# jtstrader/mercer-research

Measured on AMD Instinct MI355X. Metric: training images/sec, MNIST-shape 28x28x1 batch=256, at 1/2/4/8 MI355X, higher is better.
Workload: dtype f32

## Files before the change

mercer_research_amd/csrc/dense_xcd.hpp:

```cpp
#pragma once

#include "dense_p2.hpp"
#include "dense_p2_dp.hpp"
#include "dp_push.hpp"

namespace rcn {

constexpr int kXcdWorkers = 32, kXcdThreads = 512, kXcdFlagStride = 32;
constexpr int kXcdSl = 2;

template <typename T>
struct XcdBufsT {
    T* slab;
    T* d1;
    T* a1;
    T* d2;
    T* loss;
    T* a2;
    T* d3;
    T* fragimg;
    unsigned* flagA;
    unsigned* flagB;
    unsigned* flagT;
    unsigned* xcc;
    unsigned* flagD;
    unsigned* errd;
    unsigned* done;
    unsigned* cw;
    unsigned* cdone;
    long long* phase;
};
using XcdBufs = XcdBufsT<float>;

inline int xcd_na(const NetDesc& nd) { return (pipe_slices(nd) + kXcdSl - 1) / kXcdSl; }
inline bool xcd_two_hidden(const NetDesc& nd) {
    return nd.L == 3 && nd.dims[1] <= kP2H && nd.dims[2] <= kP2C && nd.dims[3] <= kP2C && pipe_slices(nd) <= kP2MaxSlices;
}
inline bool xcd_one_hidden(const NetDesc& nd) {
    return nd.L == 2 && nd.dims[1] <= kP2H && nd.dims[2] <= kP2C && pipe_slices(nd) <= kP2MaxSlices;
}
constexpr int kXcdMaxB = 256;
constexpr int kXcdMaxB64 = 256;
inline int xcd_max_b(size_t esz) { return esz == 8 ? kXcdMaxB64 : kXcdMaxB; }
inline int xcd_bt(size_t B) { return B <= 32 ? 32 : B <= 64 ? 64 : B <= 128 ? 128 : 256; }
inline bool xcd_supported(const NetDesc& nd, size_t B, size_t esz = 4) {
    return (xcd_one_hidden(nd) || xcd_two_hidden(nd)) && B >= 1 && B <= (size_t)xcd_max_b(esz) && xcd_na(nd) + pipe_extra_wgs(nd) <= kXcdWorkers &&
           pipe_extra_wgs(nd) <= 8;
}
inline int xcd_workers(const NetDesc& nd, int BT) {
    const int roles = xcd_na(nd) + pipe_extra_wgs(nd), groups = BT / kP2Ts;
    return roles > groups ? roles : groups;
}
inline size_t xcd_buf_bytes(const NetDesc& nd, size_t BT, size_t esz = 4) {
    const size_t NS = BT / kP2Ts, NA = (size_t)xcd_na(nd);
    return (NS * NA * kP2Ts * kP2H + 2 * BT * kP2H + 3 * BT * kP2C + NS + (size_t)kP3BFrag * 64) * esz +
           (size_t)(4 * kXcdWorkers + 8) * kXcdFlagStride * sizeof(unsigned) + 512 + 1024;
}
constexpr int kXcdD1Ld = 48;
template <typename T, int BT> constexpr bool xcd_red_aliased() { return sizeof(T) == 8 && BT >= 128; }
template <typename T, int BT> constexpr bool xcd_single_buffer() { return sizeof(T) == 8 && BT >= 256; }
constexpr size_t xcd_lds_floats(int BT, bool red_aliased = false, bool single = false) {
    return (single ? 1 : 2) * (size_t)kXcdSl * BT * 16 + (size_t)(single ? BT / 2 : BT) * kXcdD1Ld + (red_aliased ? 0 : (size_t)kDenseWaves * kMtp * kRedTile) +
           (size_t)kXcdSl * 16 * kP2H + (size_t)kP2BWaves * 64 * 4 + kP2H * kLd + 3 * kP2C * kLd + 4 * 64 + 64;
}
template <typename T, int BT> constexpr size_t xcd_lds_bytes() { return xcd_lds_floats(BT, xcd_red_aliased<T, BT>(), xcd_single_buffer<T, BT>()) * sizeof(T); }
static_assert(xcd_lds_bytes<double, 128>() + 64 <= 160 * 1024 && xcd_lds_bytes<float, 256>() + 64 <= 160 * 1024 && xcd_lds_bytes<double, 256>() + 64 <= 160 * 1024,
              "k_xcd_epoch: LDS of the largest instantiations");
static_assert((size_t)2 * kXcdSl * 128 * 16 >= (size_t)kDenseWaves * kMtp * kRedTile, "k_xcd_epoch: the partials fit the batch buffers they are laid over");

#ifdef RCN_STAMPS
#define XSTAMP(i) do { if (j == nb - 2 && lane == 0) g_rcn_stamps[0][w][i] = __builtin_amdgcn_s_memrealtime(); } while (0)
#define XCLOCK(k) do { if (lane == 0 && wave == 0) { g_rcn_stamps[1][w][2 * (k)] = __builtin_amdgcn_s_memtime(); g_rcn_stamps[1][w][2 * (k) + 1] = __builtin_amdgcn_s_memrealtime(); } } while (0)
#else
#define XSTAMP(i) do { } while (0)
#define XCLOCK(k) do { } while (0)
#endif
#if defined(RCN_STAMPS) && defined(RCN_STAMPS_TAIL)
#define XSTAMP_TAIL(i) XSTAMP(i)
#define XSTAMP_FWD(i) do { } while (0)
#else
#define XSTAMP_TAIL(i) do { } while (0)
#define XSTAMP_FWD(i) XSTAMP(i)
#endif

using xu4 = __attribute__((ext_vector_type(4))) unsigned;
#define XCD_RSRC(ptr, bytes) __builtin_amdgcn_make_buffer_rsrc((void*)(ptr), 0, (int)(bytes), 0x00020000)
template <typename T> __device__ inline typename Vec4<T>::type xcd_ld4(__amdgpu_buffer_rsrc_t r, int byte_off);
template <> __device__ inline Vec4<float>::type xcd_ld4<float>(__amdgpu_buffer_rsrc_t r, int byte_off) {
    const xu4 v = __builtin_amdgcn_raw_buffer_load_b128(r, byte_off, 0, 16);
    Vec4<float>::type f;
    __builtin_memcpy(&f, &v, 16);
    return f;
}
template <> __device__ inline Vec4<double>::type xcd_ld4<double>(__amdgpu_buffer_rsrc_t r, int byte_off) {
    const xu4 v[2] = {__builtin_amdgcn_raw_buffer_load_b128(r, byte_off, 0, 16), __builtin_amdgcn_raw_buffer_load_b128(r, byte_off + 16, 0, 16)};
    Vec4<double>::type f;
    __builtin_memcpy(&f, v, 32);
    return f;
}
__device__ inline float xcd_ld1_at(__amdgpu_buffer_rsrc_t r, int lane_off, int uniform_off) {
    const unsigned v = __builtin_amdgcn_raw_buffer_load_b32(r, lane_off, uniform_off, 16);
    float f;
    __builtin_memcpy(&f, &v, 4);
    return f;
}
template <typename T> __device__ inline T xcd_ld1(__amdgpu_buffer_rsrc_t r, int byte_off);
template <> __device__ inline float xcd_ld1<float>(__amdgpu_buffer_rsrc_t r, int byte_off) {
    const unsigned v = __builtin_amdgcn_raw_buffer_load_b32(r, byte_off, 0, 16);
    float f;
    __builtin_memcpy(&f, &v, 4);
    return f;
}
template <> __device__ inline double xcd_ld1<double>(__amdgpu_buffer_rsrc_t r, int byte_off) {
    typedef unsigned xu2 __attribute__((ext_vector_type(2)));
    const xu2 v = __builtin_amdgcn_raw_buffer_load_b64(r, byte_off, 0, 16);
    double f;
    __builtin_memcpy(&f, &v, 8);
    return f;
}
__device__ inline void xcd_drain() { asm volatile("s_waitcnt vmcnt(0)" ::: "memory"); }
__device__ inline void xcd_flag(unsigned* f, unsigned tag) { __hip_atomic_store(f, tag, __ATOMIC_RELAXED, __HIP_MEMORY_SCOPE_WORKGROUP); }
__device__ inline void xcd_flag_wt(unsigned* f, unsigned v) { __hip_atomic_store(f, v, __ATOMIC_RELAXED, __HIP_MEMORY_SCOPE_AGENT); }

enum XcdSite : unsigned {
    kXcdSitePlacement = 1,
    kXcdSiteTailFlag = 2,
    kXcdSiteSlabFlag = 3,
    kXcdSiteDeltaFlag = 4,
    kXcdSitePushOwner = 5,
    kXcdSitePushMember = 6,
    kXcdSitePushTail = 7,
    kXcdSitePushCost = 8,
    kXcdSiteClosing = 9,
};
constexpr int kXcdRecWords = 12;
#ifdef RCN_AB_RAISE_INLINE
__device__ inline void xcd_raise(unsigned* err_host, unsigned* err_dev, unsigned code, unsigned site, int worker, int step, unsigned launch,
                                 unsigned long long missing, unsigned tag, int rank = 0, int world = 1, int xsel = 0, int nw = 0) {
#else
__device__ __attribute__((noinline)) void xcd_raise(unsigned* err_host, unsigned* err_dev, unsigned code, unsigned site, int worker, int step, unsigned launch,
                                                    unsigned long long missing, unsigned tag, int rank = 0, int world = 1, int xsel = 0, int nw = 0) {
#endif
    unsigned expect = 0u;
    if (!__hip_atomic_compare_exchange_strong(err_dev, &expect, code, __ATOMIC_RELAXED, __ATOMIC_RELAXED, __HIP_MEMORY_SCOPE_AGENT)) return;
    unsigned id;
    asm volatile("s_getreg_b32 %0, hwreg(HW_REG_XCC_ID)" : "=s"(id));
    const unsigned rec[kXcdRecWords] = {site, (unsigned)worker, (unsigned)step, launch & 0x3fffffffu, (unsigned)missing, (unsigned)(missing >> 32), tag, id & 0xfu,
                                        (unsigned)rank, (unsigned)world, (unsigned)xsel, (unsigned)nw};
#pragma unroll
    for (int i = 0; i < kXcdRecWords; ++i) __hip_atomic_store(err_host + 4 + i, rec[i], __ATOMIC_RELAXED, __HIP_MEMORY_SCOPE_SYSTEM);
    __hip_atomic_store(err_host, code, __ATOMIC_RELEASE, __HIP_MEMORY_SCOPE_SYSTEM);
}

__device__ inline void xcd_barrier_lds() { asm volatile("s_waitcnt lgkmcnt(0)\n\ts_barrier" ::: "memory"); }

__device__ inline unsigned long long xcd_wait(const unsigned* f0, int n0, const unsigned* f1, int n1, unsigned tag, long long timeout, const unsigned* err) {
    const int lane = threadIdx.x & 63;
    const unsigned* p = lane < n0 ? f0 + lane * kXcdFlagStride : (lane < n0 + n1 ? f1 + (lane - n0) * kXcdFlagStride : nullptr);
    long long t0 = 0;
    for (unsigned it = 0;; ++it) {
        const unsigned f = p ? __hip_atomic_load(p, __ATOMIC_RELAXED, __HIP_MEMORY_SCOPE_AGENT) : tag;
        if (__all((int)(f - tag) >= 0)) return 0ull;
        if ((it & 255u) == 255u) {
            const long long now = wall_clock64();
            if (t0 == 0) t0 = now;
            else if (now - t0 > timeout || __hip_atomic_load(err, __ATOMIC_RELAXED, __HIP_MEMORY_SCOPE_AGENT) != 0u) return __ballot((int)(f - tag) < 0);
        }
    }
}
__device__ inline unsigned long long xcd_wait_some(const unsigned* f0, int first, int stride, int n, unsigned tag, long long timeout, const unsigned* err) {
    const int prod = first + (int)(threadIdx.x & 63) * stride;
    const unsigned* p = prod < n ? f0 + prod * kXcdFlagStride : nullptr;
    long long t0 = 0;
    for (unsigned it = 0;; ++it) {
        const unsigned f = p ? __hip_atomic_load(p, __ATOMIC_RELAXED, __HIP_MEMORY_SCOPE_AGENT) : tag;
        if (__all((int)(f - tag) >= 0)) return 0ull;
        if ((it & 255u) == 255u) {
            const long long now = wall_clock64();
            if (t0 == 0) t0 = now;
            else if (now - t0 > timeout || __hip_atomic_load(err, __ATOMIC_RELAXED, __HIP_MEMORY_SCOPE_AGENT) != 0u) return __ballot((int)(f - tag) < 0);
        }
    }
}
__device__ inline unsigned long long xcd_missing(unsigned long long lanes, int first, int stride) {
    unsigned long long missing = 0ull;
    for (; lanes; lanes &= lanes - 1ull) missing |= 1ull << (first + __builtin_ctzll(lanes) * stride);
    return missing;
}
struct XcdTopMiss { unsigned site; unsigned long long producers; };
__host__ __device__ constexpr XcdTopMiss xcd_top_missing(unsigned long long lanes, int na, int nt) {
    const unsigned long long slab = lanes & ((1ull << na) - 1ull), tail = (lanes >> na) & ((1ull << nt) - 1ull);
    return slab != 0ull ? XcdTopMiss{kXcdSiteSlabFlag, slab} : XcdTopMiss{kXcdSiteTailFlag, tail};
}
static_assert(xcd_top_missing(0x2ull, 25, 3).site == kXcdSiteSlabFlag && xcd_top_missing(0x2ull, 25, 3).producers == 0x2ull, "only a slab part missing");
static_assert(xcd_top_missing(5ull << 25, 25, 3).site == kXcdSiteTailFlag && xcd_top_missing(5ull << 25, 25, 3).producers == 0x5ull, "only tail tiles missing, NT = 3");
static_assert(xcd_top_missing((4ull << 25) | 0x1000002ull, 25, 3).site == kXcdSiteSlabFlag && xcd_top_missing((4ull << 25) | 0x1000002ull, 25, 3).producers == 0x1000002ull,
              "both missing: the slab site, the slab producers only");
static_assert(xcd_top_missing(0x21ull << 25, 25, 6).site == kXcdSiteTailFlag && xcd_top_missing(0x21ull << 25, 25, 6).producers == 0x21ull, "tail tiles 0 and 5 of NT = 6");
static_assert(xcd_top_missing(0x3full << 2, 2, 6).site == kXcdSiteTailFlag && xcd_top_missing(0x3full << 2, 2, 6).producers == 0x3full, "every tail tile of NT = 6 behind NA = 2");
static_assert(xcd_top_missing((1ull << 31) | 1ull, 29, 3).site == kXcdSiteSlabFlag && xcd_top_missing((1ull << 31) | 1ull, 29, 3).producers == 1ull, "NA = 29: the last tail lane is lane 31");
static_assert(xcd_top_missing(1ull << 28, 29, 3).site == kXcdSiteSlabFlag && xcd_top_missing(1ull << 29, 29, 3).site == kXcdSiteTailFlag &&
              xcd_top_missing(1ull << 29, 29, 3).producers == 1ull, "the boundary between the two tables");

constexpr unsigned kXcdPoison = 0x10000u;
__device__ inline bool xcd_commit(unsigned* cw, int NW, long long timeout, const unsigned* err, bool& gave_up, unsigned& seen) {
    unsigned v = __hip_atomic_fetch_add(cw, 1u, __ATOMIC_RELAXED, __HIP_MEMORY_SCOPE_AGENT) + 1u;
    long long t0 = 0;
    gave_up = false;
    for (unsigned it = 0;; ++it) {
        if (v & kXcdPoison) { seen = v; return false; }
        if ((int)(v & 0xffffu) == NW) { seen = v; return true; }
        if ((it & 63u) == 63u) {
            const long long now = wall_clock64();
            if (t0 == 0) t0 = now;
            else if (now - t0 > timeout || __hip_atomic_load(err, __ATOMIC_RELAXED, __HIP_MEMORY_SCOPE_AGENT) != 0u) {
                for (;;) {
                    if (v & kXcdPoison) { seen = v; return false; }
                    if ((int)(v & 0xffffu) == NW) { seen = v; return true; }
                    unsigned expect = v;
                    if (__hip_atomic_compare_exchange_strong(cw, &expect, v | kXcdPoison, __ATOMIC_RELAXED, __ATOMIC_RELAXED, __HIP_MEMORY_SCOPE_AGENT)) {
                        gave_up = true;
                        seen = v;
                        return false;
                    }
                    v = expect;
                }
            }
        }
        __builtin_amdgcn_s_sleep(1);
        v = __hip_atomic_load(cw, __ATOMIC_RELAXED, __HIP_MEMORY_SCOPE_AGENT);
    }
}

__device__ inline void xcd_frag_scatter2(int jl, int cc, int m, int H, float v, float* __restrict__ img) { p2_frag_scatter(jl, cc, m, H, v, img); }
__device__ inline void xcd_frag_scatter3(int cc, int m, int H2, float v, float* __restrict__ img) { p3_frag_scatter(cc, m, H2, v, img); }
__device__ inline void xcd_frag_scatter2(int jl, int cc, int m, int H, double v, double* __restrict__ img) {
    if (jl == 1 && cc < H) {
        const int h = cc, c = m;
        img[(h >> 2) * 64 + (h & 3) * 16 + c] = v;
        img[(8 + (h >> 4) * 4 + (c >> 2)) * 64 + (c & 3) * 16 + (h & 15)] = v;
    } else if (jl == 1) {
        const int c = m;
#pragma unroll
        for (int nn = 0; nn < 16; ++nn) img[(16 + (c >> 2)) * 64 + (c & 3) * 16 + nn] = v;
    } else {
        const int h = m;
#pragma unroll
        for (int s = 0; s < 8; ++s) img[(24 + (h & 3)) * 64 + (h >> 2) + 8 * s] = v;
    }
}
__device__ inline void xcd_frag_scatter3(int cc, int m, int H2, double v, double* __restrict__ img) {
    if (cc < H2) {
        const int h2 = cc, c = m;
        img[(28 + (h2 >> 2)) * 64 + (h2 & 3) * 16 + c] = v;
        img[(32 + (c >> 2)) * 64 + (c & 3) * 16 + h2] = v;
    } else {
        const int c = m;
#pragma unroll
        for (int nn = 0; nn < 16; ++nn) img[(36 + (c >> 2)) * 64 + (c & 3) * 16 + nn] = v;
    }
}

__device__ inline float xcd_sigmoid(float x) { return sigmoid_fast(x); }
__device__ inline double xcd_sigmoid(double x) {
    double t = -x;
    t = t < -708.0 ? -708.0 : (t > 708.0 ? 708.0 : t);
    const double n = __builtin_rint(t * 1.44269504088896338700e+00);
    double r = __builtin_fma(n, -6.93147180369123816490e-01, t);
    r = __builtin_fma(n, -1.90821492927058770002e-10, r);
    double p = 1.0 / 6227020800.0;
    p = __builtin_fma(p, r, 1.0 / 479001600.0);
    p = __builtin_fma(p, r, 1.0 / 39916800.0);
    p = __builtin_fma(p, r, 1.0 / 3628800.0);
    p = __builtin_fma(p, r, 1.0 / 362880.0);
    p = __builtin_fma(p, r, 1.0 / 40320.0);
    p = __builtin_fma(p, r, 1.0 / 5040.0);
    p = __builtin_fma(p, r, 1.0 / 720.0);
    p = __builtin_fma(p, r, 1.0 / 120.0);
    p = __builtin_fma(p, r, 1.0 / 24.0);
    p = __builtin_fma(p, r, 1.0 / 6.0);
    p = __builtin_fma(p, r, 0.5);
    p = __builtin_fma(p, r, 1.0);
    p = __builtin_fma(p, r, 1.0);
    const double d = 1.0 + __builtin_ldexp(p, (int)n);
    double y = __builtin_amdgcn_rcp(d);
    y = __builtin_fma(__builtin_fma(-d, y, 1.0), y, y);
    y = __builtin_fma(__builtin_fma(-d, y, 1.0), y, y);
    return y;
}

struct XcdDpOn { PushDesc pd; unsigned seq0; long long ptimeout; };
struct XcdDpOff {};
template <bool DP> struct XcdDpSel { using type = XcdDpOff; };
template <> struct XcdDpSel<true> { using type = XcdDpOn; };
template <bool DP> using XcdDpArgs = typename XcdDpSel<DP>::type;

template <typename T, int BT, bool FULL, bool DP, bool L3 = false, bool GA = false, bool PH = false>
__global__ __launch_bounds__(kXcdThreads) void k_xcd_epoch(
    NetDesc nd, T* __restrict__ params, const T* __restrict__ xs_all, const T* __restrict__ ys_all, int B_arg, int nb, int G, T scale,
    T loss_scale, T* __restrict__ loss_dev, XcdBufsT<T> bufs, unsigned tag0, unsigned* __restrict__ err, long long timeout, XcdDpArgs<DP> dp,
    int xsel, const int* __restrict__ gperm, unsigned launch_id) {
    constexpr bool gather = GA;
    const int B = FULL ? BT : B_arg;
    static_assert(!GA || FULL, "the gather form exists for the full batch only");
    static_assert(BT == 32 || BT == 64 || BT == 128 || BT == 256, "k_xcd_epoch: batch instantiations");
    static_assert(!GA || BT == 256, "the gather form exists for batch 256 only");
    static_assert(sizeof(T) == 4 || (!DP && !GA && BT <= kXcdMaxB64), "f64: single-GPU forms on the packed image");
    constexpr bool SB = xcd_single_buffer<T, BT>();
    constexpr int DH = SB ? 2 : 1, BH = BT / DH;
    constexpr bool kWaveWaits = sizeof(T) == 4 && !PH && BT >= 64;
    constexpr bool kLateCopy = sizeof(T) == 4 && !PH && !SB && BT >= 64;
    constexpr bool kLatePrefetch = sizeof(T) == 4 && !PH && !SB && !DP && BT >= 64;
    constexpr bool kLateTargets = kLatePrefetch;
    constexpr bool kGatherAhead = GA && kLatePrefetch;
#ifdef RCN_AB_TWO_TOP_WAITS
    constexpr bool kOneTopWait = false;
#else
    constexpr bool kOneTopWait = kLatePrefetch;
#endif
#ifdef RCN_AB_NO_TAIL_COST
    constexpr bool kTailCost = false;
#else
    constexpr bool kTailCost = kLatePrefetch;
#endif
#ifdef RCN_AB_NO_WORDS_BY_USE
    constexpr bool kTailWordsByUse = false;
#else
    constexpr bool kTailWordsByUse = kOneTopWait;
#endif
    static_assert(!PH || DP, "the phase clocks exist for the data-parallel form");
    constexpr int ES = (int)sizeof(T), VS = 4 * ES;
    constexpr int RI = sizeof(T) == 4 ? 1 : 4;
    constexpr size_t kXs = (size_t)kXcdSl * BT * 16;
    constexpr int NS = BT / kP2Ts;
    using acc_t = typename Mfma16<T>::acc_t;
    using vec4 = typename Vec4<T>::type;
    unsigned my_xcc;
    asm volatile("s_getreg_b32 %0, hwreg(HW_REG_XCC_ID)" : "=s"(my_xcc));
    my_xcc &= 0xfu;
    if (xsel < 8 ? (int)(blockIdx.x & 7) != xsel : (int)my_xcc != xsel - 8) return;
    const int w = (int)(blockIdx.x >> 3);
    const int F = nd.dims[0], H = nd.dims[1], Cm = nd.dims[2], C = nd.dims[L3 ? 3 : 2];
    const int NA = (G + kXcdSl - 1) / kXcdSl, NT = 1 + nd.tile_start[nd.L] - nd.tile_start[1];
    const int NW = NA + NT > NS ? NA + NT : NS;
    if (w >= NW) return;
    extern __shared__ __attribute__((aligned(16))) unsigned char smem_dyn[];
    __shared__ int s_abort;
    T* smem = reinterpret_cast<T*>(smem_dyn);
    T* xbuf = smem;
    T* d1s = xbuf + (SB ? 1 : 2) * kXs;
    constexpr bool RA = xcd_red_aliased<T, BT>();
    T* red = RA ? xbuf : d1s + BH * kXcdD1Ld;
    T* wsl = d1s + BH * kXcdD1Ld + (RA ? 0 : kDenseWaves * kMtp * kRedTile);
    vec4* zred = reinterpret_cast<vec4*>(wsl + kXcdSl * 16 * kP2H);
    T* a1s = reinterpret_cast<T*>(zred) + kP2BWaves * 64 * 4;
    T* d2s = a1s + kP2H * kLd;
    T* frag = d2s + kP2C * kLd;
    T* a2s = frag + 4 * 64;
    T* d3s = a2s + kP2C * kLd;

    const int tid = threadIdx.x, wave = tid >> 6, lane = tid & 63, n = lane & 15, g4 = lane >> 4;
    const bool is_a = w < NA, is_t = w >= NA && w < NA + NT, is_s = w < NS;
    int dp_rank = 0, dp_world = 1;
    if constexpr (DP) { dp_rank = dp.pd.pd.rank; dp_world = dp.pd.pd.world; }
    const int e = w - NA;
    const int nsl = is_a ? (G - kXcdSl * w < kXcdSl ? G - kXcdSl * w : kXcdSl) : 0;
    const size_t xs_stride = (size_t)G * B * 16, ys_stride = (size_t)B * C;
    const auto r_slab = XCD_RSRC(bufs.slab, (size_t)NS * NA * kP2Ts * kP2H * ES);
    const auto r_d1 = XCD_RSRC(bufs.d1, (size_t)BT * kP2H * ES), r_a1 = XCD_RSRC(bufs.a1, (size_t)BT * kP2H * ES);
    const auto r_d2 = XCD_RSRC(bufs.d2, (size_t)BT * kP2C * ES), r_loss = XCD_RSRC(bufs.loss, (size_t)NS * ES);
    const auto r_img = XCD_RSRC(bufs.fragimg, (size_t)(L3 ? kP3BFrag : kP2BFrag) * 64 * ES);
    const auto r_a2 = XCD_RSRC(bufs.a2, (size_t)BT * kP2C * ES), r_d3 = XCD_RSRC(bufs.d3, (size_t)BT * kP2C * ES);

    if (tid == 0) s_abort = 0;
    __syncthreads();
    const unsigned vtag = launch_id & 0x00ffffffu;
    if (tid == 0) {
        const unsigned id = ((blockIdx.x & 7u) << 4) | my_xcc;
        xcd_flag(bufs.flagA + w * kXcdFlagStride, tag0 - 1u);
        xcd_flag(bufs.flagB + w * kXcdFlagStride, tag0 - 1u);
        xcd_flag(bufs.flagD + w * kXcdFlagStride, tag0 - 1u);
        if (w < 8) xcd_flag(bufs.flagT + w * kXcdFlagStride, tag0 - 1u);
        if (w == 0) __hip_atomic_store(bufs.cw, 0u, __ATOMIC_RELAXED, __HIP_MEMORY_SCOPE_AGENT);
        xcd_drain();
        xcd_flag_wt(bufs.xcc + w * kXcdFlagStride, (vtag << 8) | id);
    }
    if (wave == 0) {
        long long t0 = 0;
        bool ok = true;
        unsigned mine = 0, v = 0;
        const bool stale = __hip_atomic_load(bufs.errd, __ATOMIC_RELAXED, __HIP_MEMORY_SCOPE_AGENT) != 0u;
        if (stale && lane == 0) s_abort = 1;
        if (!stale)
        for (unsigned it = 0;; ++it) {
            v = lane < NW ? __hip_atomic_load(bufs.xcc + lane * kXcdFlagStride, __ATOMIC_RELAXED, __HIP_MEMORY_SCOPE_AGENT) : (vtag << 8);
            if (__all((v >> 8) == vtag)) break;
            if ((it & 255u) == 255u) {
                const long long now = wall_clock64();
                if (t0 == 0) t0 = now;
                else if (now - t0 > timeout || __hip_atomic_load(bufs.errd, __ATOMIC_RELAXED, __HIP_MEMORY_SCOPE_AGENT) != 0u) { ok = false; break; }
            }
            __builtin_amdgcn_s_sleep(2);
        }
        mine = __shfl(v, w < 64 ? w : 0, 64) & 0xffu;
        const bool same = __all(lane >= NW || (v & 0xffu) == mine);
        const unsigned long long absent = ok ? __ballot(lane < NW && (v & 0xffu) != mine) : __ballot(lane < NW && (v >> 8) != vtag);
        if (lane == 0 && !stale && !(ok && same)) {
            s_abort = 1;
            xcd_raise(err, bufs.errd, ok ? 2u : 1u, kXcdSitePlacement, w, -1, launch_id, absent, vtag, dp_rank, dp_world, xsel, NW);
        }
    }
    __syncthreads();
    if (s_abort) return;
    if ((launch_id >> 31) != 0u && w == 1) return;
    const bool late_closer = ((launch_id >> 30) & 1u) != 0u && w == 1;

    auto xrow4 = [&](int b, int i) -> vec4 {
        const int sl = i >> 10, smp = (i >> 2) & 255, col = (kXcdSl * w + sl) * 16 + 4 * (i & 3);
        const unsigned at = (unsigned)(b * B + smp);
        const unsigned row = gperm ? (unsigned)gperm[at] : at;
        const vec4 v = *reinterpret_cast<const vec4*>(xs_all + (size_t)row * F + (col < F ? col : 0));
        return (sl < nsl && col < F) ? v : vec4{0, 0, 0, 0};
    };
    static_assert(!GA || (kXcdThreads == 512 && kXcdSl == 2), "the gather form's element map");
    unsigned grow[2] = {0u, 0u};
    auto gidx = [&](int b, unsigned (&g)[2]) {
#pragma unroll
        for (int k = 0; k < 2; ++k) {
            const unsigned at = (unsigned)(b * B + (tid >> 2) + 128 * k);
            g[k] = gperm ? (unsigned)gperm[at] : at;
        }
    };
    auto grows4 = [&](const unsigned (&g)[2], vec4 (&x)[4]) {
#pragma unroll
        for (int r = 0; r < 4; ++r) {
            const int sl = r >> 1, col = (kXcdSl * w + sl) * 16 + 4 * (tid & 3);
            const vec4 v = *reinterpret_cast<const vec4*>(xs_all + (size_t)g[r & 1] * F + (col < F ? col : 0));
            x[r] = (sl < nsl && col < F) ? v : vec4{0, 0, 0, 0};
        }
    };
    T* W0 = params + nd.w_off[0];
    const int mt = tid >> 8;
    const int tl = wave & 3, kh = wave >> 2, usl = tl >> 1, umt = tl & 1;
    T wcur[4] = {0, 0, 0, 0};
    bool wvalid[4] = {false, false, false, false};
    unsigned woff0 = 0;
    if (is_a) {
        if (kh == 0) {
            const int f0 = (kXcdSl * w + usl) * 16;
            const int nf = usl < nsl ? (F - f0 < 16 ? F - f0 : 16) : 0;
#pragma unroll
            for (int i = 0; i < 4; ++i) {
                const int hid = umt * 16 + Mfma16<T>::row(lane, i);
                wvalid[i] = hid < H && n < nf;
                if (i == 0) woff0 = wvalid[0] ? (unsigned)((f0 + n) * H + hid) : 0u;
                const T v = W0[wvalid[i] ? woff0 + RI * i : 0u];
                wcur[i] = wvalid[i] ? v : (T)0;
            }
            store4<T>(wsl + (usl * 16 + n) * kP2H + umt * 16, lane, acc_t{wcur[0], wcur[1], wcur[2], wcur[3]});
        }
        if constexpr (kGatherAhead) {
            unsigned g0[2] = {0u, 0u}, g1[2] = {0u, 0u};
            gidx(0, g0);
            if (nb > 1) gidx(1, g1);
            if (nb > 2) gidx(2, grow);
            vec4 x0[4], x1[4];
            grows4(g0, x0);
            if (nb > 1) grows4(g1, x1);
            vec4* dst = reinterpret_cast<vec4*>(xbuf);
#pragma unroll
            for (int r = 0; r < 4; ++r) dst[tid + r * kXcdThreads] = x0[r];
            if (nb > 1) {
                dst = reinterpret_cast<vec4*>(xbuf + kXs);
#pragma unroll
                for (int r = 0; r < 4; ++r) dst[tid + r * kXcdThreads] = x1[r];
            }
        } else
        for (int b = 0; b < (SB ? 1 : 2) && b < nb; ++b) {
            vec4* dst = reinterpret_cast<vec4*>(xbuf + (size_t)(b & 1) * kXs);
            if constexpr (gather) {
                for (int i = tid; i < kXcdSl * BT * 4; i += kXcdThreads) dst[i] = xrow4(b, i);
            } else {
                const vec4* src = reinterpret_cast<const vec4*>(xs_all + (size_t)b * xs_stride + (size_t)(kXcdSl * w) * B * 16);
                for (int i = tid; i < kXcdSl * BT * 4; i += kXcdThreads) {
                    const int sl = i / (BT * 4), r = i % (BT * 4);
                    dst[i] = (sl < nsl && (r >> 2) < B) ? src[sl * B * 4 + r] : vec4{0, 0, 0, 0};
                }
            }
        }
    }
    T tcur = 0;
    size_t tp = 0;
    bool tvalid = false;
    const int nt1 = nd.tile_start[2] - nd.tile_start[1];
    auto tile_of = [&](int& jl, int& n0) {
        if (e == 0) { jl = 0; n0 = F; }
        else if (!L3 || e - 1 < nt1) { jl = 1; n0 = (e - 1) * 16; }
        else { jl = 2; n0 = (e - 1 - nt1) * 16; }
    };
    if (is_t) {
        int jl, n0;
        tile_of(jl, n0);
        const int Kin = nd.dims[jl], M = nd.dims[jl + 1];
        const int o = tid & 255, tm = mt * 16 + (o & 15), cc = n0 + (o >> 4);
        tvalid = tm < M && cc <= Kin;
        tp = tvalid ? (size_t)nd.w_off[jl] + (size_t)cc * M + tm : 0;
        tcur = params[tp];
    }
    __syncthreads();

    auto nothing = [] {};
    auto forward = [&](int jn, auto&& behind_stores) {
        const T* xb = xbuf + (SB ? (size_t)0 : (size_t)(jn & 1) * kXs);
        constexpr int NTILE = BT / 16, UT = NTILE > kDenseWaves ? NTILE / kDenseWaves : 1;
        T wf[kXcdSl][4][kMtp];
#pragma unroll
        for (int sl = 0; sl < kXcdSl; ++sl)
#pragma unroll
            for (int i = 0; i < 4; ++i)
#pragma unroll
                for (int t = 0; t < kMtp; ++t) wf[sl][i][t] = wsl[(sl * 16 + 4 * g4 + i) * kP2H + t * 16 + n];
        if (NTILE >= kDenseWaves || wave < NTILE)
#pragma unroll
        for (int u = 0; u < UT; ++u) {
            const int s = 16 * (wave + 8 * u) + n;
            vec4 xv[kXcdSl];
#pragma unroll
            for (int sl = 0; sl < kXcdSl; ++sl) xv[sl] = *reinterpret_cast<const vec4*>(xb + ((size_t)sl * BT + s) * 16 + 4 * g4);
            acc_t acc[kMtp];
#pragma unroll
            for (int t = 0; t < kMtp; ++t) acc[t] = acc_t{0, 0, 0, 0};
#pragma unroll
            for (int sl = 0; sl < kXcdSl; ++sl)
#pragma unroll
                for (int i = 0; i < 4; ++i)
#pragma unroll
                    for (int t = 0; t < kMtp; ++t) acc[t] = Mfma16<T>::mfma(wf[sl][i][t], xv[sl][i], acc[t]);
            T* dst = bufs.slab + (((size_t)(s >> 3) * NA + w) * kP2Ts + (s & 7)) * kP2H;
#pragma unroll
            for (int t = 0; t < kMtp; ++t) store4<T>(dst + t * 16, lane, acc[t]);
        }
        behind_stores();
        xcd_drain();
    };

    if (is_a) {
        forward(0, nothing);
        __syncthreads();
        if (tid == 0) xcd_flag(bufs.flagA + w * kXcdFlagStride, tag0);
    } else if (is_t) {
        if (tvalid) {
            int jl, n0;
            tile_of(jl, n0);
            const int o = tid & 255;
            if (L3 && jl == 2) xcd_frag_scatter3(n0 + (o >> 4), mt * 16 + (o & 15), Cm, tcur, bufs.fragimg);
            else xcd_frag_scatter2(jl, n0 + (o >> 4), mt * 16 + (o & 15), H, tcur, bufs.fragimg);
        }
        xcd_drain();
        __syncthreads();
        if (tid == 0) xcd_flag(bufs.flagT + e * kXcdFlagStride, tag0);
    }

    const bool live = n < kP2Ts && (FULL || w * kP2Ts + n < B);
    unsigned yrow = 0;
    if (gather) {
        const unsigned at = (unsigned)(w * kP2Ts + (n & 7));
        yrow = gperm ? (unsigned)gperm[at] : at;
    }
    T ynext[4] = {0, 0, 0, 0};
    auto targets = [&](int jb) {
        const int s0 = w * kP2Ts;
        const int srow = (FULL || s0 + (n & 7) < B) ? s0 + (n & 7) : B - 1;
        const T* Ys = gather ? ys_all + (size_t)yrow * C : ys_all + (size_t)jb * ys_stride + (size_t)srow * C;
#pragma unroll
        for (int i = 0; i < 4; ++i) {
            const int c = Mfma16<T>::row(lane, i);
            ynext[i] = Ys[c < C ? c : 0];
        }
        if (gather && jb + 1 < nb) {
            const unsigned at = (unsigned)((jb + 1) * B + s0 + (n & 7));
            yrow = gperm ? (unsigned)gperm[at] : at;
        }
    };
    if constexpr (kLateTargets) { if (is_s && wave == 6) targets(0); }
    long long ph_x = 0, ph_t0 = 0;
    if constexpr (PH) { if (tid == 0) ph_t0 = wall_clock64(); }
    for (int j = 0; j < nb; ++j) {
        const unsigned tag = tag0 + (unsigned)j;
        if (j == 8) XCLOCK(0);
        if (j == nb - 8) XCLOCK(1);
        const bool more = j + 1 < nb;
        constexpr int XR = (kXcdSl * BT * 4 + kXcdThreads - 1) / kXcdThreads;
        vec4 xr[XR];
        const bool pre = is_a && (SB ? j + 1 < nb : j + 2 < nb);
        auto prefetch = [&](int jb) {
            const vec4* src = reinterpret_cast<const vec4*>(xs_all + (size_t)jb * xs_stride + (size_t)(kXcdSl * w) * B * 16);
#pragma unroll
            for (int r = 0; r < XR; ++r) {
                const int i = tid + r * kXcdThreads, sl = i / (BT * 4), rr = i % (BT * 4);
                xr[r] = (sl < nsl && (rr >> 2) < B) ? src[sl * B * 4 + rr] : vec4{0, 0, 0, 0};
            }
        };
        if constexpr (!kLatePrefetch)
        if (pre && !SB) {
            if constexpr (gather) {
#pragma unroll
                for (int r = 0; r < XR; ++r) xr[r] = xrow4(j + 2, tid + r * kXcdThreads);
            } else {
                const vec4* src = reinterpret_cast<const vec4*>(xs_all + (size_t)(j + 2) * xs_stride + (size_t)(kXcdSl * w) * B * 16);
                if (FULL) {
#pragma unroll
                    for (int r = 0; r < XR; ++r) {
                        const int i = tid + r * kXcdThreads;
                        xr[r] = i < nsl * BT * 4 ? src[i] : vec4{0, 0, 0, 0};
                    }
                } else {
#pragma unroll
                    for (int r = 0; r < XR; ++r) {
                        const int i = tid + r * kXcdThreads, sl = i / (BT * 4), rr = i % (BT * 4);
                        xr[r] = (sl < nsl && (rr >> 2) < B) ? src[sl * B * 4 + rr] : vec4{0, 0, 0, 0};
                    }
                }
            }
        }

        if (is_s) {
            const int s0 = w * kP2Ts;
            const int srow = (FULL || s0 + (n & 7) < B) ? s0 + (n & 7) : B - 1;
            const T* Ys = gather ? ys_all + (size_t)yrow * C
                                 : ys_all + (size_t)j * ys_stride + (size_t)srow * C;
            T fr[L3 ? kP3BFrag : kP2BFrag];
            if (wave == 0) {
                XSTAMP(0);
                if constexpr (kOneTopWait) {
                    const unsigned long long mAT = xcd_wait(bufs.flagA, NA, bufs.flagT, NT, tag, timeout, bufs.errd);
                    if (mAT != 0ull && lane == 0) {
                        const XcdTopMiss miss = xcd_top_missing(mAT, NA, NT);
                        s_abort = 1;
                        xcd_raise(err, bufs.errd, 1u, miss.site, w, j, launch_id, miss.producers, tag, dp_rank, dp_world, xsel, NW);
                    }
                } else {
                const unsigned long long mT = xcd_wait(bufs.flagT, NT, nullptr, 0, tag, timeout, bufs.errd);
#pragma unroll
                for (int q = 0; q < (L3 ? kP3BFrag : kP2BFrag); ++q) fr[q] = (q >= 20 && q < 24) ? (T)0 : xcd_ld1<T>(r_img, (q * 64 + lane) * ES);
                const unsigned long long mA = mT ? 0ull : xcd_wait(bufs.flagA, NA, nullptr, 0, tag, timeout, bufs.errd);
                if ((mT | mA) != 0ull && lane == 0) {
                    s_abort = 1;
                    xcd_raise(err, bufs.errd, 1u, mT ? kXcdSiteTailFlag : kXcdSiteSlabFlag, w, j, launch_id, mT ? mT : mA, tag, dp_rank, dp_world, xsel, NW);
                }
                }
                XSTAMP(1);
            } else if (wave == 6) {
                if constexpr (kLateTargets) {
#pragma unroll
                    for (int i = 0; i < 4; ++i) frag[i * 64 + lane] = ynext[i];
                } else {
#pragma unroll
                for (int i = 0; i < 4; ++i) {
                    const int c = Mfma16<T>::row(lane, i);
                    frag[i * 64 + lane] = Ys[c < C ? c : 0];
                }
                if (gather && more) {
                    const unsigned at = (unsigned)((j + 1) * B + s0 + (n & 7));
                    yrow = gperm ? (unsigned)gperm[at] : at;
                }
                }
            }
            __syncthreads();
// ... 72 lines not shown
                {
                    const int s = lane >> 3, h0 = 4 * (lane & 7);
                    vec4 a;
#pragma unroll
                    for (int i = 0; i < 4; ++i) {
                        const auto sg = xcd_sigmoid(z[i] + fr[24 + i]);
                        a[i] = (h0 + i < H) ? sg : (T)0;
                        a1s[(h0 + i) * kLd + s] = a[i];
                    }
                    *reinterpret_cast<vec4*>(bufs.a1 + (size_t)(s0 + s) * kP2H + h0) = a;
                }
                XSTAMP_TAIL(14);
                acc_t acc = acc_t{0, 0, 0, 0};
                {
                    T bv[8];
#pragma unroll
                    for (int ks = 0; ks < 8; ++ks) bv[ks] = a1s[(4 * ks + g4) * kLd + (n & 7)];
#pragma unroll
                    for (int ks = 0; ks < 8; ++ks) acc = Mfma16<T>::mfma(fr[ks], n < kP2Ts ? bv[ks] : (T)0, acc);
                }
                T lsum = 0;
                [[maybe_unused]] const bool want_cost = loss_dev != nullptr || DP;
                auto cost_share = [&] {
                    lsum = wave_sum_lane0(lsum);
                    if (lane == 0) bufs.loss[w] = lsum;
                };
                acc_t dv;
                if constexpr (!L3) {
#pragma unroll
                    for (int i = 0; i < 4; ++i) {
                        const int c = Mfma16<T>::row(lane, i);
                        const T a2 = xcd_sigmoid(acc[i] + fr[16 + i]);
                        const T diff = a2 - fr[20 + i];
                        const bool ok = c < C && live;
                        dv[i] = ok ? diff * (a2 * ((T)1 - a2)) : (T)0;
                        lsum += ok ? diff * diff : (T)0;
                        d2s[c * kLd + n] = dv[i];
                    }
                } else {
                    acc_t a2r;
#pragma unroll
                    for (int i = 0; i < 4; ++i) {
                        const int h2 = Mfma16<T>::row(lane, i);
                        const T a = xcd_sigmoid(acc[i] + fr[16 + i]);
                        a2r[i] = (h2 < Cm && n < kP2Ts) ? a : (T)0;
                        a2s[h2 * kLd + n] = a2r[i];
                    }
                    if (n < kP2Ts) store4<T>(bufs.a2 + (size_t)(s0 + n) * kP2C, lane, a2r);
                    acc_t acc3 = acc_t{0, 0, 0, 0};
                    {
                        T bv[4];
#pragma unroll
                        for (int ks = 0; ks < 4; ++ks) bv[ks] = a2s[(4 * ks + g4) * kLd + (n & 7)];
#pragma unroll
                        for (int ks = 0; ks < 4; ++ks) acc3 = Mfma16<T>::mfma(fr[28 + ks], n < kP2Ts ? bv[ks] : (T)0, acc3);
                    }
                    acc_t d3v;
#pragma unroll
                    for (int i = 0; i < 4; ++i) {
                        const int c = Mfma16<T>::row(lane, i);
                        const T a3 = xcd_sigmoid(acc3[i] + fr[36 + i]);
                        const T diff = a3 - fr[20 + i];
                        const bool ok = c < C && live;
                        d3v[i] = ok ? diff * (a3 * ((T)1 - a3)) : (T)0;
                        lsum += ok ? diff * diff : (T)0;
                        d3s[c * kLd + n] = d3v[i];
                    }
                    if (n < kP2Ts) store4<T>(bufs.d3 + (size_t)(s0 + n) * kP2C, lane, d3v);
                    acc_t ad2 = acc_t{0, 0, 0, 0};
                    {
                        T dvv[4];
#pragma unroll
                        for (int ks = 0; ks < 4; ++ks) dvv[ks] = d3s[(4 * ks + g4) * kLd + n];
#pragma unroll
                        for (int ks = 0; ks < 4; ++ks) ad2 = Mfma16<T>::mfma(fr[32 + ks], dvv[ks], ad2);
                    }
#pragma unroll
                    for (int i = 0; i < 4; ++i) {
                        const int h2 = Mfma16<T>::row(lane, i);
                        dv[i] = ad2[i] * (a2r[i] * ((T)1 - a2r[i]));
                        d2s[h2 * kLd + n] = dv[i];
                    }
                }
                XSTAMP_TAIL(15);
                if (n < kP2Ts) store4<T>(bufs.d2 + (size_t)(s0 + n) * kP2C, lane, dv);
                {
                    T dvv[4], av[kMtp][4];
#pragma unroll
                    for (int ks = 0; ks < 4; ++ks) dvv[ks] = d2s[(4 * ks + g4) * kLd + n];
#pragma unroll
                    for (int t = 0; t < kMtp; ++t)
#pragma unroll
                        for (int i = 0; i < 4; ++i) av[t][i] = a1s[(t * 16 + Mfma16<T>::row(lane, i)) * kLd + (n & 7)];
                    if constexpr (kTailCost) { if (want_cost) cost_share(); }
#pragma unroll
                    for (int t = 0; t < kMtp; ++t) {
                        acc_t ad = acc_t{0, 0, 0, 0};
#pragma unroll
                        for (int ks = 0; ks < 4; ++ks) ad = Mfma16<T>::mfma(fr[8 + t * 4 + ks], dvv[ks], ad);
                        acc_t o;
#pragma unroll
                        for (int i = 0; i < 4; ++i) o[i] = ad[i] * (av[t][i] * ((T)1 - av[t][i]));
                        if (n < kP2Ts) store4<T>(bufs.d1 + (size_t)(s0 + n) * kP2H + t * 16, lane, o);
                    }
                }
                if constexpr (!kTailCost) cost_share();
                XSTAMP(4);
                xcd_drain();
                if (lane == 0) xcd_flag(bufs.flagB + w * kXcdFlagStride, tag);
                XSTAMP(5);
            }
        }

        bool waited = true;
        if constexpr (kWaveWaits) {
            if (is_a || is_t) {
                int g0 = wave, gs = kXcdThreads / 64, gn = NS;
                if (is_t) {
                    const int kc = wave * (BT >> 3);
                    g0 = kc >> 3; gs = 1; gn = ((kc + (BT >> 3) - 1) >> 3) + 1;
                    if (e == 0 && wave == 0 && (loss_dev || DP)) { g0 = 0; gn = NS; }
                }
                const unsigned long long mB = xcd_wait_some(bufs.flagB, g0, gs, gn, tag, timeout, bufs.errd);
                waited = mB == 0ull;
                if (!waited && lane == 0) {
                    s_abort = 1;
                    xcd_raise(err, bufs.errd, 1u, kXcdSiteDeltaFlag, w, j, launch_id, xcd_missing(mB, g0, gs), tag, dp_rank, dp_world, xsel, NW);
                }
                if (wave == 1) XSTAMP(6);
            } else {
                __syncthreads();
                if (s_abort) return;
            }
        } else {
            if (is_a || is_t) {
                if (wave == 1) {
                    const unsigned long long mB = xcd_wait(bufs.flagB, NS, nullptr, 0, tag, timeout, bufs.errd);
                    if (mB != 0ull && lane == 0) {
                        s_abort = 1;
                        xcd_raise(err, bufs.errd, 1u, kXcdSiteDeltaFlag, w, j, launch_id, mB, tag, dp_rank, dp_world, xsel, NW);
                    }
                }
            }
            if (wave == 1) XSTAMP(6);
            __syncthreads();
            if (s_abort) return;
            if (wave == 1) XSTAMP(7);
        }

        if (is_a) {
            acc_t acc0 = acc_t{0, 0, 0, 0}, acc1 = acc_t{0, 0, 0, 0};
#pragma unroll
            for (int dh = 0; dh < DH; ++dh) {
            {
                constexpr int DR = (BH * 8 + kXcdThreads - 1) / kXcdThreads;
                vec4 dv[DR];
#pragma unroll
                for (int r = 0; r < DR; ++r) dv[r] = xcd_ld4<T>(r_d1, (dh * BH * 8 + tid + r * kXcdThreads) * VS);
#pragma unroll
                for (int r = 0; r < DR; ++r) {
                    const int idx = tid + r * kXcdThreads;
                    if (BH * 8 >= kXcdThreads || idx < BH * 8) *reinterpret_cast<vec4*>(d1s + (idx >> 3) * kXcdD1Ld + (idx & 7) * 4) = dv[r];
                }
            }
            if (kWaveWaits && wave == 1 && dh == 0) XSTAMP(7);
            __syncthreads();
            if (kWaveWaits && dh == 0 && s_abort) return;
            if (wave == 1 && dh == 0) XSTAMP(8);
            if constexpr (SB) { if (dh == 0 && pre) prefetch(j + 1); }
            if constexpr (kLatePrefetch) {
                if (pre) {
                    if constexpr (kGatherAhead) {
                        grows4(grow, xr);
                        if (j + 3 < nb) gidx(j + 3, grow);
                    } else if constexpr (FULL) {
                        const vec4* src = reinterpret_cast<const vec4*>(xs_all + (size_t)(j + 2) * xs_stride + (size_t)(kXcdSl * w) * B * 16);
#pragma unroll
                        for (int r = 0; r < XR; ++r) {
                            const int i = tid + r * kXcdThreads;
                            xr[r] = i < nsl * BT * 4 ? src[i] : vec4{0, 0, 0, 0};
                        }
                    } else {
                        prefetch(j + 2);
                    }
                }
            }
            if (kh == 0) {
                const T* xb = xbuf + (SB ? (size_t)0 : (size_t)(j & 1) * kXs) + (size_t)usl * BT * 16 + (size_t)dh * BH * 16;
                constexpr int NQB = BH / 32;
                const T* ap = d1s + g4 * kXcdD1Ld + umt * 16 + n;
                const T* bp = xb + g4 * 16 + n;
                T av[2][8], bv[2][8];
#pragma unroll
                for (int q = 0; q < 8; ++q) { av[0][q] = ap[4 * q * kXcdD1Ld]; bv[0][q] = bp[4 * q * 16]; }
#pragma unroll
                for (int qb = 0; qb < NQB; ++qb) {
                    if (qb + 1 < NQB) {
#pragma unroll
                        for (int q = 0; q < 8; ++q) {
                            av[(qb + 1) & 1][q] = ap[4 * (8 * (qb + 1) + q) * kXcdD1Ld];
                            bv[(qb + 1) & 1][q] = bp[4 * (8 * (qb + 1) + q) * 16];
                        }
                    }
                    __builtin_amdgcn_sched_barrier(0);
#pragma unroll
                    for (int q = 0; q < 8; q += 2) {
                        acc0 = Mfma16<T>::mfma(av[qb & 1][q], bv[qb & 1][q], acc0);
                        acc1 = Mfma16<T>::mfma(av[qb & 1][q + 1], bv[qb & 1][q + 1], acc1);
                    }
                    __builtin_amdgcn_sched_barrier(0);
                }
            }
            if (dh + 1 < DH) __syncthreads();
            }
            if (kh == 0) {
                T gsum[4];
#pragma unroll
                for (int i = 0; i < 4; ++i) gsum[i] = acc0[i] + acc1[i];
                if constexpr (DP) {
                    const unsigned seq = dp.seq0 + (unsigned)j;
                    unsigned wo = woff0;
                    asm volatile("" : "+v"(wo));
                    const size_t i0 = (size_t)nd.w_off[0] + wo;
                    const bool gw[4] = {wvalid[0], wvalid[1], wvalid[2], wvalid[3]};
                    unsigned pmiss = 0u;
                    long long ph0 = 0;
                    if constexpr (PH) { if (tid == 0) ph0 = wall_clock64(); }
                    const bool ok = push_reduce4(dp.pd, w, seq, i0, gw, gsum, dp.ptimeout, &pmiss);
                    if constexpr (PH) { if (tid == 0) ph_x += wall_clock64() - ph0; }
                    if (!ok) {
                        s_abort = 1;
                        xcd_raise(err, bufs.errd, 1u, push_owner_of(w, dp_world) == dp_rank ? kXcdSitePushOwner : kXcdSitePushMember, w, j, launch_id,
                                  (unsigned long long)pmiss | ((unsigned long long)i0 << 32), seq, dp_rank, dp_world, xsel, NW);
                    }
                }
#pragma unroll
                for (int i = 0; i < 4; ++i) {
                    const T wn = wcur[i] - scale * gsum[i];
                    wcur[i] = wvalid[i] ? wn : (T)0;
                }
                store4<T>(wsl + (usl * 16 + n) * kP2H + umt * 16, lane, acc_t{wcur[0], wcur[1], wcur[2], wcur[3]});
                if (wave == 1) XSTAMP(9);
            }
            if constexpr (DP) xcd_barrier_lds(); else __syncthreads();
            if (DP && s_abort) return;
            if (wave == 1) XSTAMP(10);
            if constexpr (!kLateCopy) {
                if (pre) {
                    vec4* dst = reinterpret_cast<vec4*>(xbuf + (SB ? (size_t)0 : (size_t)(j & 1) * kXs));
#pragma unroll
                    for (int r = 0; r < XR; ++r)
                        if (kXcdSl * BT * 4 >= kXcdThreads || tid + r * kXcdThreads < kXcdSl * BT * 4) dst[tid + r * kXcdThreads] = xr[r];
                }
            }
            if constexpr (SB) __syncthreads();
            if (more) {
                if constexpr (kLateCopy) {
                    forward(j + 1, [&]() {
                        if (pre) {
                            vec4* dst = reinterpret_cast<vec4*>(xbuf + (size_t)(j & 1) * kXs);
#pragma unroll
                            for (int r = 0; r < XR; ++r)
                                if (kXcdSl * BT * 4 >= kXcdThreads || tid + r * kXcdThreads < kXcdSl * BT * 4) dst[tid + r * kXcdThreads] = xr[r];
                        }
                    });
                } else {
                    forward(j + 1, nothing);
                }
                if (wave == 1) XSTAMP(11);
                if (wave == 0) XSTAMP_FWD(13);
                if (wave == 4) XSTAMP_FWD(14);
                if (wave == 7) XSTAMP_FWD(15);
                __syncthreads();
                if (tid == 0) xcd_flag(bufs.flagA + w * kXcdFlagStride, tag + 1);
                if (wave == 0) XSTAMP(12);
            }
        } else if (is_t) {
            if (e == 0 && wave == 0 && (loss_dev || DP) && waited) {
                T t = lane < NS ? xcd_ld1<T>(r_loss, lane * ES) : (T)0;
#pragma unroll
                for (int sh = 16; sh >= 1; sh >>= 1) t += __shfl_xor(t, sh, 64);
                t *= loss_scale;
                if (lane == 0) {
                if constexpr (DP) {
                    const unsigned seq = dp.seq0 + (unsigned)j;
                    T g = t;
                    unsigned pmiss = 0u;
                    if (dp.pd.pd.world == 1 || push_all1(dp.pd, seq, (size_t)nd.P, t, dp.ptimeout, g, &pmiss)) t = g;
                    else { s_abort = 1; xcd_raise(err, bufs.errd, 1u, kXcdSitePushCost, w, j, launch_id, (unsigned long long)pmiss | ((unsigned long long)nd.P << 32), seq, dp_rank, dp_world, xsel, NW); }
                }
                if (loss_dev) loss_dev[j] = t;
                }
            }
            int jl, n0;
            tile_of(jl, n0);
            const int Kin = nd.dims[jl], M = nd.dims[jl + 1];
            const int c = n0 + n;
            const auto r_act = e == 0 ? r_d1 : ((L3 && jl == 2) ? r_a2 : r_a1);
            const auto r_del = e == 0 ? r_d1 : ((L3 && jl == 2) ? r_d3 : r_d2);
            const int ldD = e == 0 ? kP2H : kP2C, ldA = (L3 && jl == 2) ? kP2C : kP2H;
            acc_t acc[kMtp];
#pragma unroll
            for (int t = 0; t < kMtp; ++t) acc[t] = acc_t{0, 0, 0, 0};
            {
                constexpr int NQ = BT / 32;
                const int kc = wave * (BT >> 3);
                const int cc_ld = (e != 0 && c < Kin) ? c : 0;
                T bv[NQ], av[NQ][kMtp];
#pragma unroll
                for (int q = 0; q < NQ; ++q) {
                    const int s = kc + 4 * q + g4;
                    bv[q] = xcd_ld1<T>(r_act, (int)(((size_t)s * ldA + cc_ld) * ES));
#pragma unroll
                    for (int t = 0; t < kMtp; ++t) {
                        const int row = t * 16 + n;
                        av[q][t] = xcd_ld1<T>(r_del, (int)(((size_t)s * ldD + (row < M ? row : M - 1)) * ES));
                    }
                }
                __builtin_amdgcn_sched_barrier(0);
#pragma unroll
                for (int q = 0; q < NQ; ++q) {
                    const T b = (e != 0 && c < Kin) ? bv[q] : (c == Kin ? (T)1 : (T)0);
#pragma unroll
                    for (int t = 0; t < kMtp; ++t) acc[t] = Mfma16<T>::mfma(t * 16 + n < M ? av[q][t] : (T)0, b, acc[t]);
                }
            }
            store_partials<T>(red, wave, lane, acc);
            __syncthreads();
            if (kWaveWaits && s_abort) return;
            {
                const int o = tid & 255, tcl = o >> 4, tml = o & 15, tm = mt * 16 + tml, cc = n0 + tcl;
                if (tvalid) {
                    T gsum = sum_partials<T>(red, mt, tcl, tml);
                    if constexpr (DP) {
                        const unsigned seq = dp.seq0 + (unsigned)j;
                        size_t tpo = tp;
                        asm volatile("" : "+v"(tpo));
                        T g = gsum;
                        unsigned pmiss = 0u;
                        long long ph0 = 0;
                        if constexpr (PH) { if (tid == 0) ph0 = wall_clock64(); }
                        const bool pok = dp.pd.pd.world == 1 || push_all1(dp.pd, seq, tpo, gsum, dp.ptimeout, g, &pmiss);
                        if constexpr (PH) { if (tid == 0) ph_x += wall_clock64() - ph0; }
                        if (pok) gsum = g;
                        else { s_abort = 1; xcd_raise(err, bufs.errd, 1u, kXcdSitePushTail, w, j, launch_id, (unsigned long long)pmiss | ((unsigned long long)tpo << 32), seq, dp_rank, dp_world, xsel, NW); }
                    }
                    tcur -= scale * gsum;
                    int tmo = tm;
                    asm volatile("" : "+v"(tmo));
                    if (L3 && jl == 2) xcd_frag_scatter3(cc, tmo, Cm, tcur, bufs.fragimg);
                    else xcd_frag_scatter2(jl, cc, tmo, H, tcur, bufs.fragimg);
                }
            }
            xcd_drain();
            __syncthreads();
            if (DP && s_abort) return;
            if (more && tid == 0) xcd_flag(bufs.flagT + e * kXcdFlagStride, tag + 1);
            if (wave == 0) XSTAMP(12);
        }
    }

    if constexpr (PH) {
        if (tid == 0) {
            bufs.phase[w * 4 + 0] = ph_x;
            bufs.phase[w * 4 + 1] = wall_clock64() - ph_t0;
            bufs.phase[w * 4 + 2] = nb;
            bufs.phase[w * 4 + 3] = is_a ? (push_owner_of(w, dp_world) == dp_rank ? 1 : 2) : (is_t ? 3 : 0);
        }
    }
    {
        const unsigned tagD = tag0 + (unsigned)nb - 1u;
        __syncthreads();
        if (tid == 0) {
            if (late_closer) {
                const long long t0 = wall_clock64();
                while (wall_clock64() - t0 < 3 * timeout) __builtin_amdgcn_s_sleep(8);
            }
            xcd_flag(bufs.flagD + w * kXcdFlagStride, tagD);
            bool gave_up;
            unsigned seen;
            const bool commit = xcd_commit(bufs.cw, NW, timeout, bufs.errd, gave_up, seen);
            if (!commit) {
                s_abort = 1;
                if (gave_up) xcd_raise(err, bufs.errd, 1u, kXcdSiteClosing, w, nb - 1, launch_id, (unsigned long long)(seen & 0xffffu), tagD, dp_rank, dp_world, xsel, NW);
            }
        }
        __syncthreads();
        if (s_abort) return;
        if (w == 0 && tid == 0) __hip_atomic_store(bufs.done, launch_id & 0x3fffffffu, __ATOMIC_RELAXED, __HIP_MEMORY_SCOPE_SYSTEM);
    }
    if (is_a) {
#pragma unroll
        for (int i = 0; i < 4; ++i)
// ... 19 lines not shown
```

Measured before the change: 43.14 million.

## Load d1 via buffer-to-LDS DMA with swizzle; store W0 slice hidden-major

The d1 gradient tile is now loaded straight from global memory into LDS with buffer_load_lds, using an XOR-swizzled 32-word row layout instead of staging it through registers. The d1 region moves to the front of LDS so its pieces are aligned. The per-worker W0 slice is also stored hidden-major with a swizzle, so the forward pass can read it with conflict-free b128 loads. Compile-time asserts check the bank maps. The risk is added drain waits and extra scattered b32 stores on the weight update.

```diff
diff --git a/mercer_research_amd/csrc/dense_xcd.hpp b/mercer_research_amd/csrc/dense_xcd.hpp
--- a/mercer_research_amd/csrc/dense_xcd.hpp
+++ b/mercer_research_amd/csrc/dense_xcd.hpp
@@ -57,6 +57,75 @@
            (size_t)(4 * kXcdWorkers + 8) * kXcdFlagStride * sizeof(unsigned) + 512 + 1024;
 }
 constexpr int kXcdD1Ld = 48;
+constexpr int kXcdD1DmaLd = 32;
+constexpr int xcd_d1_src_byte(int row0, int L) { return (row0 + (L >> 3)) * 128 + (((L & 7) ^ (4 * ((row0 + (L >> 3)) & 1))) << 4); }
+constexpr int xcd_d1_word(int row, int h) { return row * kXcdD1DmaLd + ((((h >> 2)) ^ (4 * (row & 1))) << 2) + (h & 3); }
+constexpr bool xcd_d1_piece_ok(int row0) {
+    unsigned long long seen = 0ull;
+    for (int L = 0; L < 64; ++L) {
+        const int src = xcd_d1_src_byte(row0, L) - row0 * 128;
+        if (src < 0 || src >= 1024 || (src & 15) != 0) return false;
+        seen |= 1ull << (src >> 4);
+        const int row = row0 + (L >> 3), c = (src >> 4) & 7;
+        if ((src >> 7) != (L >> 3)) return false;
+        for (int k = 0; k < 4; ++k)
+            if (xcd_d1_word(row, 4 * c + k) != row0 * kXcdD1DmaLd + 4 * L + k) return false;
+    }
+    return seen == ~0ull;
+}
+constexpr bool xcd_d1_read_ok(int r, int umt) {
+    unsigned banks0 = 0u, banks1 = 0u;
+    for (int n = 0; n < 16; ++n) {
+        banks0 |= 1u << (xcd_d1_word(r, umt * 16 + n) & 31);
+        banks1 |= 1u << (xcd_d1_word(r + 1, umt * 16 + n) & 31);
+    }
+    return (banks0 & banks1) == 0u && __builtin_popcount(banks0) == 16 && __builtin_popcount(banks1) == 16;
+}
+static_assert(xcd_d1_piece_ok(0) && xcd_d1_piece_ok(8) && xcd_d1_piece_ok(64 + 56) && xcd_d1_piece_ok(192 + 56), "kD1Dma: a piece's source map");
+static_assert(xcd_d1_read_ok(0, 0) && xcd_d1_read_ok(0, 1) && xcd_d1_read_ok(1, 0) && xcd_d1_read_ok(1, 1) && xcd_d1_read_ok(2, 0) && xcd_d1_read_ok(3, 1) &&
+              xcd_d1_read_ok(254, 0) && xcd_d1_read_ok(254, 1), "kD1Dma: rows r, r + 1 of one operand read land on disjoint banks");
+constexpr int kXcdW0Ld = 32;
+constexpr int xcd_w0_word(int h, int f) { return h * kXcdW0Ld + ((((f >> 2)) ^ ((h >> 1) & 7)) << 2) + (f & 3); }
+constexpr bool xcd_w0_read_ok(int sl, int t) {
+    constexpr unsigned long long sets[4] = {0x000000000ff0f00full, 0x00000000f00f0ff0ull, 0x0ff0f00f00000000ull, 0xf00f0ff000000000ull};
+    for (int s = 0; s < 4; ++s) {
+        unsigned quads = 0u;
+        for (int lane = 0; lane < 64; ++lane)
+            if ((sets[s] >> lane) & 1ull) {
+                const int wd = xcd_w0_word(16 * t + (lane & 15), 16 * sl + 4 * (lane >> 4));
+                if ((wd & 3) != 0) return false;
+                quads |= 1u << ((wd >> 2) & 15);
+            }
+        if (quads != 0xffffu) return false;
+    }
+    return true;
+}
+constexpr bool xcd_w0_write_ok(int usl, int umt, int i) {
+    for (int half = 0; half < 2; ++half) {
+        int hits[32] = {};
+        for (int l = 0; l < 32; ++l) {
+            const int lane = 32 * half + l;
+            if (++hits[xcd_w0_word(16 * umt + 4 * (lane >> 4) + i, 16 * usl + (lane & 15)) & 31] > 2) return false;
+        }
+    }
+    return true;
+}
+constexpr bool xcd_w0_bijective() {
+    for (int h = 0; h < 32; ++h) {
+        unsigned seen = 0u;
+        for (int f = 0; f < 32; ++f) {
+            const int wd = xcd_w0_word(h, f);
+            if (wd / kXcdW0Ld != h) return false;
+            seen |= 1u << (wd % kXcdW0Ld);
+        }
+        if (seen != 0xffffffffu) return false;
+    }
+    return true;
+}
+static_assert(xcd_w0_bijective(), "kW0ByHidden: the image's map");
+static_assert(xcd_w0_read_ok(0, 0) && xcd_w0_read_ok(0, 1) && xcd_w0_read_ok(1, 0) && xcd_w0_read_ok(1, 1), "kW0ByHidden: the forward's b128 reads are conflict-free");
+static_assert(xcd_w0_write_ok(0, 0, 0) && xcd_w0_write_ok(0, 0, 1) && xcd_w0_write_ok(0, 0, 2) && xcd_w0_write_ok(0, 0, 3) && xcd_w0_write_ok(1, 1, 0) &&
+              xcd_w0_write_ok(1, 1, 1) && xcd_w0_write_ok(1, 0, 2) && xcd_w0_write_ok(0, 1, 3), "kW0ByHidden: the gradient's b32 stores are at most 2-way");
 template <typename T, int BT> constexpr bool xcd_red_aliased() { return sizeof(T) == 8 && BT >= 128; }
 template <typename T, int BT> constexpr bool xcd_single_buffer() { return sizeof(T) == 8 && BT >= 256; }
 constexpr size_t xcd_lds_floats(int BT, bool red_aliased = false, bool single = false) {
@@ -328,6 +397,16 @@
 #else
     constexpr bool kTailWordsByUse = kOneTopWait;
 #endif
+#ifdef RCN_AB_NO_D1_DMA
+    constexpr bool kD1Dma = false;
+#else
+    constexpr bool kD1Dma = kLatePrefetch;
+#endif
+#ifdef RCN_AB_NO_W0_BY_HIDDEN
+    constexpr bool kW0ByHidden = false;
+#else
+    constexpr bool kW0ByHidden = kLatePrefetch;
+#endif
     static_assert(!PH || DP, "the phase clocks exist for the data-parallel form");
     constexpr int ES = (int)sizeof(T), VS = 4 * ES;
     constexpr int RI = sizeof(T) == 4 ? 1 : 4;
@@ -347,11 +426,12 @@
     extern __shared__ __attribute__((aligned(16))) unsigned char smem_dyn[];
     __shared__ int s_abort;
     T* smem = reinterpret_cast<T*>(smem_dyn);
-    T* xbuf = smem;
-    T* d1s = xbuf + (SB ? 1 : 2) * kXs;
+    T* xbuf = kD1Dma ? smem + BH * kXcdD1Ld : smem;
+    T* d1s = kD1Dma ? smem : xbuf + (SB ? 1 : 2) * kXs;
+    T* past_d1 = smem + (SB ? 1 : 2) * kXs + BH * kXcdD1Ld;
     constexpr bool RA = xcd_red_aliased<T, BT>();
-    T* red = RA ? xbuf : d1s + BH * kXcdD1Ld;
-    T* wsl = d1s + BH * kXcdD1Ld + (RA ? 0 : kDenseWaves * kMtp * kRedTile);
+    T* red = RA ? xbuf : past_d1;
+    T* wsl = past_d1 + (RA ? 0 : kDenseWaves * kMtp * kRedTile);
     vec4* zred = reinterpret_cast<vec4*>(wsl + kXcdSl * 16 * kP2H);
     T* a1s = reinterpret_cast<T*>(zred) + kP2BWaves * 64 * 4;
     T* d2s = a1s + kP2H * kLd;
@@ -457,6 +537,10 @@
                 const T v = W0[wvalid[i] ? woff0 + RI * i : 0u];
                 wcur[i] = wvalid[i] ? v : (T)0;
             }
+            if constexpr (kW0ByHidden) {
+#pragma unroll
+                for (int i = 0; i < 4; ++i) wsl[xcd_w0_word(umt * 16 + 4 * g4 + i, usl * 16 + n)] = wcur[i];
+            } else
             store4<T>(wsl + (usl * 16 + n) * kP2H + umt * 16, lane, acc_t{wcur[0], wcur[1], wcur[2], wcur[3]});
         }
         if constexpr (kGatherAhead) {
@@ -514,6 +598,16 @@
         const T* xb = xbuf + (SB ? (size_t)0 : (size_t)(jn & 1) * kXs);
         constexpr int NTILE = BT / 16, UT = NTILE > kDenseWaves ? NTILE / kDenseWaves : 1;
         T wf[kXcdSl][4][kMtp];
+        if constexpr (kW0ByHidden) {
+#pragma unroll
+            for (int sl = 0; sl < kXcdSl; ++sl)
+#pragma unroll
+                for (int t = 0; t < kMtp; ++t) {
+                    const vec4 q = *reinterpret_cast<const vec4*>(wsl + xcd_w0_word(t * 16 + n, sl * 16 + 4 * g4));
+#pragma unroll
+                    for (int i = 0; i < 4; ++i) wf[sl][i][t] = q[i];
+                }
+        } else
 #pragma unroll
         for (int sl = 0; sl < kXcdSl; ++sl)
 #pragma unroll
@@ -892,7 +986,17 @@
             acc_t acc0 = acc_t{0, 0, 0, 0}, acc1 = acc_t{0, 0, 0, 0};
 #pragma unroll
             for (int dh = 0; dh < DH; ++dh) {
-            {
+            if constexpr (kD1Dma) {
+                constexpr int DR = BH * 8 / kXcdThreads;
+                static_assert(DR >= 1 && DR * kXcdThreads == BH * 8 && kXcdThreads == 512 && kP2H == kXcdD1DmaLd, "kD1Dma: whole 1 KB pieces, rows of 128 bytes");
+                const int voff = xcd_d1_src_byte(0, lane);
+                const int wave_u = __builtin_amdgcn_readfirstlane(wave);
+#pragma unroll
+                for (int r = 0; r < DR; ++r) {
+                    const int row0 = 8 * wave_u + 64 * r;
+                    __builtin_amdgcn_raw_ptr_buffer_load_lds(r_d1, (__attribute__((address_space(3))) void*)(d1s + row0 * kXcdD1DmaLd), 16, voff, row0 * 128, 0, 16);
+                }
+            } else {
                 constexpr int DR = (BH * 8 + kXcdThreads - 1) / kXcdThreads;
                 vec4 dv[DR];
 #pragma unroll
@@ -904,6 +1008,7 @@
                 }
             }
             if (kWaveWaits && wave == 1 && dh == 0) XSTAMP(7);
+            if constexpr (kD1Dma) xcd_drain();
             __syncthreads();
             if (kWaveWaits && dh == 0 && s_abort) return;
             if (wave == 1 && dh == 0) XSTAMP(8);
@@ -928,17 +1033,18 @@
             if (kh == 0) {
                 const T* xb = xbuf + (SB ? (size_t)0 : (size_t)(j & 1) * kXs) + (size_t)usl * BT * 16 + (size_t)dh * BH * 16;
                 constexpr int NQB = BH / 32;
-                const T* ap = d1s + g4 * kXcdD1Ld + umt * 16 + n;
+                constexpr int kD1Ld = kD1Dma ? kXcdD1DmaLd : kXcdD1Ld;
+                const T* ap = kD1Dma ? d1s + xcd_d1_word(g4, umt * 16 + n) : d1s + g4 * kXcdD1Ld + umt * 16 + n;
                 const T* bp = xb + g4 * 16 + n;
                 T av[2][8], bv[2][8];
 #pragma unroll
-                for (int q = 0; q < 8; ++q) { av[0][q] = ap[4 * q * kXcdD1Ld]; bv[0][q] = bp[4 * q * 16]; }
+                for (int q = 0; q < 8; ++q) { av[0][q] = ap[4 * q * kD1Ld]; bv[0][q] = bp[4 * q * 16]; }
 #pragma unroll
                 for (int qb = 0; qb < NQB; ++qb) {
                     if (qb + 1 < NQB) {
 #pragma unroll
                         for (int q = 0; q < 8; ++q) {
-                            av[(qb + 1) & 1][q] = ap[4 * (8 * (qb + 1) + q) * kXcdD1Ld];
+                            av[(qb + 1) & 1][q] = ap[4 * (8 * (qb + 1) + q) * kD1Ld];
                             bv[(qb + 1) & 1][q] = bp[4 * (8 * (qb + 1) + q) * 16];
                         }
                     }
@@ -979,6 +1085,10 @@
                     const T wn = wcur[i] - scale * gsum[i];
                     wcur[i] = wvalid[i] ? wn : (T)0;
                 }
+                if constexpr (kW0ByHidden) {
+#pragma unroll
+                    for (int i = 0; i < 4; ++i) wsl[xcd_w0_word(umt * 16 + 4 * g4 + i, usl * 16 + n)] = wcur[i];
+                } else
                 store4<T>(wsl + (usl * 16 + n) * kP2H + umt * 16, lane, acc_t{wcur[0], wcur[1], wcur[2], wcur[3]});
                 if (wave == 1) XSTAMP(9);
             }
```

Result: faster. 44.58 million, median of 6 (+3.3%).
